# PFLeget/cosmogp

Measured on NVIDIA B200. Metric: gp_fits_per_sec, higher is better.
Workload: dtype f64

## Files before the change

### cosmogp_b200/csrc/cgp_small64.cu

```cuda
#include <atomic>
#include "cgp_internal.h"
#include "cgp_math.cuh"

#include <math.h>
#include <stdlib.h>
#include <type_traits>

#ifndef CGP64_GRID_U
#define CGP64_GRID_U 2
#endif

namespace cgp {
namespace {

constexpr int TILE = 64;
constexpr unsigned FULL = 0xffffffffu;
constexpr double LOG_2PI = 1.8378770664093454835606594728112;
constexpr double LN2 = 0.693147180559945309417232;

__constant__ unsigned char kTri[36] = {
    0x00, 0x10, 0x11, 0x20, 0x21, 0x22, 0x30, 0x31, 0x32, 0x33, 0x40, 0x41, 0x42, 0x43, 0x44,
    0x50, 0x51, 0x52, 0x53, 0x54, 0x55, 0x60, 0x61, 0x62, 0x63, 0x64, 0x65, 0x66,
    0x70, 0x71, 0x72, 0x73, 0x74, 0x75, 0x76, 0x77};

__device__ __forceinline__ void dmma(double& c0, double& c1, double a, double b) {
  asm("mma.sync.aligned.m8n8k4.row.col.f64.f64.f64.f64 {%0,%1}, {%2}, {%3}, {%0,%1};"
      : "+d"(c0), "+d"(c1) : "d"(a), "d"(b));
}
__host__ __device__ constexpr int slot(int i, int j) { return ((i * (i + 1)) >> 1) + j; }
__device__ __forceinline__ int tile_off(int r, int c) {
  const int rho = r ^ ((r >> 1) & 1), sig = (r >> 1) & 2;
  return ((rho * 4 + ((c >> 1) ^ sig)) << 1) + (c & 1);
}

struct Lane {
  int g, t, nat, tr0, tr1;
  __device__ explicit Lane(int lane) {
    g = lane >> 2; t = lane & 3;
    nat = tile_off(g, 2 * t);
    tr0 = tile_off(2 * t, g); tr1 = tile_off(2 * t + 1, g);
  }
};
__device__ __forceinline__ double2 ld_frag(const double* tiles, int s, const Lane& L) {
  return *reinterpret_cast<const double2*>(tiles + s * TILE + L.nat);
}
__device__ __forceinline__ void st_frag(double* tiles, int s, const Lane& L, double v0, double v1) {
  *reinterpret_cast<double2*>(tiles + s * TILE + L.nat) = make_double2(v0, v1);
}
__device__ __forceinline__ double2 ld_frag_t(const double* tiles, int s, const Lane& L) {
  const double* p = tiles + s * TILE;
  return make_double2(p[L.tr0], p[L.tr1]);
}
__device__ __forceinline__ double2 ld_vec2(const double* v, int i) { return *reinterpret_cast<const double2*>(v + i); }
__device__ __forceinline__ double red_t(double v) {
  v += __shfl_xor_sync(FULL, v, 1); v += __shfl_xor_sync(FULL, v, 2); return v;
}
__device__ __forceinline__ double red_g(double v) {
  v += __shfl_xor_sync(FULL, v, 4); v += __shfl_xor_sync(FULL, v, 8); v += __shfl_xor_sync(FULL, v, 16); return v;
}

template <int DIM>
__device__ __forceinline__ double rbf_arg(const Cov& c, double ax, double ay, double bx, double by) {
  const double dx = ax - bx;
  if (DIM == 1) return dx * dx * c.h00;
  const double dy = ay - by;
  return fma(dy * c.h11, dy, fma(dx, c.h00, dy * c.h01) * dx);
}

struct DiagOut { double t0, t1, piv; int badk; };
template <int K>
__device__ __forceinline__ void diag_step(double& a0, double& a1, double& t0, double& t1, double& pivprod, int& badk,
                                          const int g, const int t) {
  constexpr int kc = K >> 1;
  const double ak = (K & 1) ? a1 : a0;
  const double d = __shfl_sync(FULL, ak, K * 4 + kc);
  if (!(d > 0.0) && badk == 0) badk = K + 1;
  const double rinv = cgp_rsqrt(d);
  pivprod *= d;
  const double lg = __shfl_sync(FULL, ak, g * 4 + kc) * rinv;
  const double lc0 = __shfl_sync(FULL, ak, (2 * t) * 4 + kc) * rinv;
  const double lc1 = __shfl_sync(FULL, ak, (2 * t + 1) * 4 + kc) * rinv;
  a0 = fma(-lg, lc0, a0); a1 = fma(-lg, lc1, a1);
  const double tk0 = __shfl_sync(FULL, t0, K * 4 + t) * rinv;
  const double tk1 = __shfl_sync(FULL, t1, K * 4 + t) * rinv;
  const double f = (g > K) ? lg : 0.0;
  const double n0 = fma(-f, tk0, t0), n1 = fma(-f, tk1, t1);
  t0 = (g == K) ? tk0 : n0; t1 = (g == K) ? tk1 : n1;
}
__device__ __noinline__ DiagOut diag_factor_impl(double a0, double a1, int g, int t) {
  double t0 = (g == 2 * t) ? 1.0 : 0.0;
  double t1 = (g == 2 * t + 1) ? 1.0 : 0.0;
  double pivprod = 1.0; int badk = 0;
  diag_step<0>(a0, a1, t0, t1, pivprod, badk, g, t); diag_step<1>(a0, a1, t0, t1, pivprod, badk, g, t);
  diag_step<2>(a0, a1, t0, t1, pivprod, badk, g, t); diag_step<3>(a0, a1, t0, t1, pivprod, badk, g, t);
  diag_step<4>(a0, a1, t0, t1, pivprod, badk, g, t); diag_step<5>(a0, a1, t0, t1, pivprod, badk, g, t);
  diag_step<6>(a0, a1, t0, t1, pivprod, badk, g, t); diag_step<7>(a0, a1, t0, t1, pivprod, badk, g, t);
  DiagOut o; o.t0 = t0; o.t1 = t1; o.piv = pivprod; o.badk = badk;
  return o;
}
__device__ __forceinline__ void diag_factor(double a0, double a1, const Lane& L,
                                            double& t0, double& t1, double& pivprod, int& badk) {
  const DiagOut o = diag_factor_impl(a0, a1, L.g, L.t);
  t0 = o.t0; t1 = o.t1; pivprod = o.piv; badk = o.badk;
}

static unsigned long long* next_ticket(cudaStream_t stream) {
  constexpr unsigned RING = 4096;
  constexpr int MAX_DEV = 16;
  static unsigned long long* ring[MAX_DEV] = {nullptr};
  static std::atomic<unsigned> idx[MAX_DEV];
  int dev = 0;
  if (cudaGetDevice(&dev) != cudaSuccess || dev < 0 || dev >= MAX_DEV) return nullptr;
  if (!ring[dev] && cudaMalloc((void**)&ring[dev], RING * sizeof(unsigned long long)) != cudaSuccess) return nullptr;
  unsigned long long* t = ring[dev] + (idx[dev].fetch_add(1) % RING);
  if (cudaMemsetAsync(t, 0, sizeof(unsigned long long), stream) != cudaSuccess) return nullptr;
  return t;
}

__host__ __device__ constexpr int n_vec64(int task) { return task == TASK_LOO ? 6 : 1; }
__host__ __device__ constexpr bool ktab64(int task, int nb) {
  return task == TASK_LOO || ((task == TASK_PREDICT || task == TASK_PREDICT_U || task == TASK_LL) && nb < 8);
}
#ifndef CGP64_GRID_WPC
#define CGP64_GRID_WPC 1
#endif
__host__ __device__ constexpr int warps_per_cta(int task) { return (task == TASK_PREDICT_F || task == TASK_PREDICT_FU) ? CGP64_GRID_WPC : 1; }

template <int DIM, int TASK, int NB>
__global__ void __launch_bounds__(32 * warps_per_cta(TASK), warps_per_cta(TASK) > 1 ? 16 / warps_per_cta(TASK) :
                                  (TASK == TASK_PREDICT || TASK == TASK_PREDICT_F || TASK == TASK_PREDICT_FU || TASK == TASK_PREDICT_U) ? 12 : 16)
gp64_kernel(const SmallArgs a, unsigned long long* __restrict__ ticket) {
  extern __shared__ __align__(16) double smem[];
  constexpr int WPC = warps_per_cta(TASK);
  const int lane = threadIdx.x & 31, warp = threadIdx.x >> 5;
  const Lane L(lane);
  Cov cov = a.cov;
  constexpr int LD = 8 * NB;
  constexpr int NT = NB * (NB + 1) / 2;
  double* tiles = smem;
  double* px = tiles + NT * TILE + warp * (DIM + 1) * LD;
  double* noise = px + DIM * LD;
  double* vr = tiles + NT * TILE + WPC * (DIM + 1) * LD;
  constexpr bool PF = TASK == TASK_PREDICT_F || TASK == TASK_PREDICT_FU;
  constexpr bool UNI = TASK == TASK_PREDICT_FU || TASK == TASK_PREDICT_U;
  constexpr bool FUSED = TASK == TASK_PREDICT || TASK == TASK_PREDICT_U;
  constexpr bool PRED_LIKE = FUSED || TASK == TASK_FACTOR || PF;
  constexpr bool NEGL = PRED_LIKE;
  double* vz = PRED_LIKE ? vr : vr + LD;
  double* va = PRED_LIKE ? vr : vz + LD;
  double* vd = va + LD;
  double* v1 = vd + LD;
  double* vu = v1 + LD;

  constexpr bool TAB = PF && !UNI && NB == 8 && WPC == 1;
  if (TAB) { exp_table_to_shared(noise, lane); __syncwarp(); }
  constexpr bool KTAB = ktab64(TASK, NB);
  double* const ktab = tiles + NT * TILE + (WPC * (DIM + 1) + n_vec64(TASK)) * LD;
  if (KTAB) { exp_table_to_shared(ktab, lane); __syncwarp(); }
  const int split = (FUSED || PF) ? a.split : 1;
  const int64_t* const part_off = (FUSED || PF) ? a.part_off : nullptr;
  const int64_t n_work = part_off ? a.n_parts : (a.n_obj_dev ? (int64_t)*a.n_obj_dev : a.n_obj) * split;
  __shared__ __align__(8) unsigned long long s_mbar;
  __shared__ long long s_tk[2];
  unsigned mbar_parity = 0;
  if (PF) {
    if (threadIdx.x == 0) {
      asm volatile("mbarrier.init.shared::cta.b64 [%0], 1;" :: "r"((unsigned)__cvta_generic_to_shared(&s_mbar)));
      asm volatile("fence.mbarrier_init.release.cluster;" ::: "memory");
    }
    if (WPC > 1) __syncthreads(); else __syncwarp();
  }

  constexpr int NR = (LD + 31) / 32;
  struct Next { int64_t o0; int n; double x[NR], y2[NR], r[NR], ye[NR]; };
  auto fetch = [&](int64_t w, Next& nx) {
    nx.n = -1;
    if (w >= n_work) return;
    int part, parts;
    const int64_t oi = work_item(part_off, a.n_obj, split, w, part, parts);
    const int64_t b = a.order ? a.order[oi] : oi;
    nx.o0 = a.off[b];
    nx.n = (int)(a.off[b + 1] - nx.o0);
#pragma unroll
    for (int k = 0; k < NR; ++k) {
      const int i = k * 32 + lane;
      const bool in = i < nx.n;
      if (DIM == 1) { nx.x[k] = in ? a.x[nx.o0 + i] : 0.0; nx.y2[k] = 0.0; }
      else { nx.x[k] = in ? a.x[2 * (nx.o0 + i)] : 0.0; nx.y2[k] = in ? a.x[2 * (nx.o0 + i) + 1] : 0.0; }
      if (PF) { nx.ye[k] = 0.0; nx.r[k] = 0.0; continue; }
      nx.ye[k] = (in && a.yerr) ? a.yerr[nx.o0 + i] : 0.0;
      nx.r[k] = in ? (a.y[nx.o0 + i] - (a.y0 ? a.y0[nx.o0 + i] : 0.0)) : 0.0;
    }
  };
  double uni_g0 = 0.0, uni_delta = 0.0, uni_c0 = 1.0, uni_c1 = 1.0, uni_c2 = 1.0, uni_2hd = 0.0;
  if (UNI) {
    uni_g0 = a.xnew[0];
    uni_delta = (a.xnew[a.m_shared - 1] - uni_g0) / (double)(a.m_shared - 1);
    const double k0 = (double)L.g * uni_delta, k1 = (double)(L.g + 8) * uni_delta;
    uni_c0 = cgp_exp(cov.h00 * k0 * k0); uni_c1 = cgp_exp(cov.h00 * k1 * k1);
    const double k2 = (double)(L.g + 16) * uni_delta;
    uni_c2 = cgp_exp(cov.h00 * k2 * k2);
    uni_2hd = 2.0 * cov.h00 * uni_delta;
  }
  int64_t w = blockIdx.x, w_nxt = (int64_t)blockIdx.x + gridDim.x, t_next = 0;
  int it = 0;
  auto advance = [&]() -> int64_t {
    if (WPC > 1) { __syncthreads(); return s_tk[(it++) & 1]; }
    return __shfl_sync(FULL, t_next, 0);
  };
  Next nx;
  fetch(w, nx);
  for (;; w = w_nxt, w_nxt = advance()) {
    if (w >= n_work) break;
    if (threadIdx.x == 0) {
      t_next = (int64_t)atomicAdd(ticket, 1ULL) + 2 * (int64_t)gridDim.x;
      if (WPC > 1) s_tk[it & 1] = t_next;
    }
    int part, parts;
    const int64_t oi = work_item(part_off, a.n_obj, split, w, part, parts);
    const int64_t b = a.order ? a.order[oi] : oi;
    const int64_t o0 = nx.o0;
    const int n = nx.n;
    const int64_t io = a.compact_io ? oi : b;
    if (a.hyp_obj) cov = cov_from_hyp(DIM, a.hyp_obj + io * a.n_hyp, a.nugget_obj ? a.nugget_obj[io] : a.nugget_shared,
                                      a.floor_shared, a.flags);

    __syncwarp();
    double rsum = 0.0;
#pragma unroll
    for (int k = 0; k < NR; ++k) {
      const int i = k * 32 + lane;
      if (i < LD) {
        px[i] = nx.x[k];
        if (DIM == 2) px[LD + i] = nx.y2[k];
        if (!PF) {
          noise[i] = nx.ye[k] * nx.ye[k] + cov.noise_const;
          vr[i] = nx.r[k]; rsum += nx.r[k];
        }
      }
    }
    double xo[NR];
#pragma unroll
    for (int k = 0; k < NR; ++k) xo[k] = UNI ? nx.x[k] : 0.0;
    fetch(w_nxt, nx);
    __syncwarp();
    if (TASK == TASK_LOO) rsum = red_g(red_t(rsum));
    double lp_m = 1.0; int lp_e = 0; int bad = 0;
    const bool want_u = (TASK == TASK_LOO) && (a.loo_mode == 1);
    if (PF) {
      const unsigned mb = (unsigned)__cvta_generic_to_shared(&s_mbar);
      if (threadIdx.x == 0) {
        const unsigned bytes = NT * TILE * 8;
        const double* src = a.fws + b * a.fws_stride;
        asm volatile("fence.proxy.async.shared::cta;" ::: "memory");
        asm volatile("mbarrier.arrive.expect_tx.shared::cta.b64 _, [%0], %1;" :: "r"(mb), "r"(bytes + LD * 8) : "memory");
        asm volatile("cp.async.bulk.shared::cluster.global.mbarrier::complete_tx::bytes [%0], [%1], %2, [%3];"
                     :: "r"((unsigned)__cvta_generic_to_shared(tiles)), "l"(src), "r"(bytes), "r"(mb) : "memory");
        asm volatile("cp.async.bulk.shared::cluster.global.mbarrier::complete_tx::bytes [%0], [%1], %2, [%3];"
                     :: "r"((unsigned)__cvta_generic_to_shared(va)), "l"(src + NT * TILE), "r"((unsigned)(LD * 8)), "r"(mb) : "memory");
      }
      bad = a.info[b];
      unsigned done = 0;
      while (!done) {
        asm volatile("{\n\t.reg .pred p;\n\tmbarrier.try_wait.parity.shared::cta.b64 p, [%1], %2;\n\tselp.u32 %0, 1, 0, p;\n\t}"
                     : "=r"(done) : "r"(mb), "r"(mbar_parity) : "memory");
      }
      mbar_parity ^= 1;
    }
    if (!PF) {

    constexpr int TPP = 4;
#pragma unroll 1
    for (int q = 0; q < NT; q += TPP) {
      double kv[TPP][2];
#pragma unroll
      for (int u = 0; u < TPP; ++u) {
        const int qq = (q + u < NT) ? q + u : q;
        const int ij = kTri[qq];
        const int I = ij >> 4, J = ij & 15;
        const int gi = 8 * I + L.g, cj = 8 * J + 2 * L.t;
        const double xi = px[gi], yi = DIM == 2 ? px[LD + gi] : 0.0;
        const double q0 = rbf_arg<DIM>(cov, xi, yi, px[cj], DIM == 2 ? px[LD + cj] : 0.0);
        const double q1 = rbf_arg<DIM>(cov, xi, yi, px[cj + 1], DIM == 2 ? px[LD + cj + 1] : 0.0);
        double e0 = KTAB ? cgp_exp_tab(q0, ktab) : cgp_exp(q0);
        double e1 = KTAB ? cgp_exp_tab(q1, ktab) : cgp_exp(q1);
        e0 = (gi < n && cj < gi) ? e0 : 0.0;
        e1 = (gi < n && cj + 1 < gi) ? e1 : 0.0;
        const double dg = (gi < n) ? cov.amp_auto + noise[gi] : 1.0;
        kv[u][0] = (cj == gi) ? dg : cov.amp_auto * e0;
        kv[u][1] = (cj + 1 == gi) ? dg : cov.amp_auto * e1;
      }
#pragma unroll
      for (int u = 0; u < TPP; ++u) {
        if (q + u < NT) st_frag(tiles, q + u, L, kv[u][0], kv[u][1]);
      }
    }
    __syncwarp();

#pragma unroll
    for (int J = 0; J < NB; ++J) {
      double s0[NB], s1[NB], u0[NB], u1[NB];
#pragma unroll
      for (int i = 0; i < NB; ++i) { s0[i] = 0.0; s1[i] = 0.0; u0[i] = 0.0; u1[i] = 0.0; }
#pragma unroll
      for (int P = 0; P < J; ++P) {
        const double2 fb = ld_frag(tiles, slot(J, P), L);
        dmma(s0[0], s1[0], fb.x, fb.x); dmma(u0[0], u1[0], fb.y, fb.y);
#pragma unroll
        for (int i = 1; i < NB - J; ++i) {
          const double2 fa = ld_frag(tiles, slot(J + i, P), L);
          dmma(s0[i], s1[i], fa.x, fb.x); dmma(u0[i], u1[i], fa.y, fb.y);
        }
      }
#pragma unroll
      for (int i = 0; i < NB - J; ++i) {
        const double2 kk = ld_frag(tiles, slot(J + i, J), L);
        s0[i] = kk.x - (s0[i] + u0[i]);
        s1[i] = kk.y - (s1[i] + u1[i]);
      }
      double t0, t1;
      {
        double piv; int badk;
        diag_factor(s0[0], s1[0], L, t0, t1, piv, badk);
        st_frag(tiles, slot(J, J), L, t0, t1);
        if (TASK == TASK_LL || TASK == TASK_FACTOR || FUSED) {
          lp_m *= piv;
          const int hi = __double2hiint(lp_m);
          const int e = ((hi >> 20) & 0x7ff) - 1023;
          lp_e += e;
          lp_m = __hiloint2double(hi - (e << 20), __double2loint(lp_m));
        }
        if (badk && bad == 0) bad = 8 * J + badk;
      }
#pragma unroll
      for (int i = 1; i < NB - J; ++i) {
        const double c0 = s0[i], c1 = s1[i];
        s0[i] = 0.0; s1[i] = 0.0; u0[i] = 0.0; u1[i] = 0.0;
        dmma(s0[i], s1[i], c0, t0); dmma(u0[i], u1[i], c1, t1);
      }
#pragma unroll
      for (int i = 1; i < NB - J; ++i) {
        if (NEGL) st_frag(tiles, slot(J + i, J), L, -s0[i] - u0[i], -s1[i] - u1[i]);
        else st_frag(tiles, slot(J + i, J), L, s0[i] + u0[i], s1[i] + u1[i]);
      }
      if (NEGL) {
        double pz = 0.0, pz2 = 0.0;
#pragma unroll
        for (int P = 0; P < J; ++P) {
          const double2 f = ld_frag(tiles, slot(J, P), L);
          const double2 rv = ld_vec2(vr, 8 * P + 2 * L.t);
          pz = fma(f.x, rv.x, pz); pz2 = fma(f.y, rv.y, pz2);
        }
        const double wv = vr[8 * J + L.g] + red_t(pz + pz2);
        double q = t0 * __shfl_sync(FULL, wv, L.t * 8) + t1 * __shfl_sync(FULL, wv, L.t * 8 + 4);
        q = red_t(q);
        if (L.t == 0) vr[8 * J + L.g] = q;
      }
      __syncwarp();
    }

    if (TASK == TASK_LL) {
      double quad = 0.0;
#pragma unroll
      for (int J = 0; J < NB; ++J) {
        double p = 0.0, p2 = 0.0;
#pragma unroll
        for (int P = 0; P < J; ++P) {
          const double2 f = ld_frag(tiles, slot(J, P), L);
          const double2 rv = ld_vec2(vr, 8 * P + 2 * L.t);
          p = fma(f.x, rv.x, p); p2 = fma(f.y, rv.y, p2);
        }
        const double wv = vr[8 * J + L.g] - red_t(p + p2);
        const double2 f = ld_frag(tiles, slot(J, J), L);
        double q = f.x * __shfl_sync(FULL, wv, L.t * 8) + f.y * __shfl_sync(FULL, wv, L.t * 8 + 4);
        q = red_t(q);
        if (L.t == 0) { vr[8 * J + L.g] = q; quad = fma(q, q, quad); }
        __syncwarp();
      }
      quad = red_g(red_t(quad));
      if (lane == 0) {
        a.info[io] = bad;
        const double logdet = log(lp_m) + (double)lp_e * LN2;
        a.ll[io] = bad ? nan("") : -0.5 * (quad + logdet + n * LOG_2PI);
      }
      continue;
    }

    if constexpr (TASK == TASK_LOO) {
#pragma unroll
    for (int I = 1; I < NB; ++I) {
      double s0[NB], s1[NB];
#pragma unroll
      for (int j = 0; j < NB; ++j) { s0[j] = 0.0; s1[j] = 0.0; }
#pragma unroll
      for (int P = 0; P < I; ++P) {
        const double2 fb = ld_frag(tiles, slot(I, P), L);
#pragma unroll
        for (int J = 0; J <= P; ++J) {
          const double2 fa = (J == P) ? ld_frag_t(tiles, slot(P, P), L) : ld_frag(tiles, slot(P, J), L);
          dmma(s0[J], s1[J], fa.x, fb.x); dmma(s0[J], s1[J], fa.y, fb.y);
        }
      }
      const double2 ft = ld_frag(tiles, slot(I, I), L);
#pragma unroll
      for (int J = 0; J < I; ++J) {
        double r0 = 0.0, r1 = 0.0, e0 = 0.0, e1 = 0.0;
        dmma(r0, r1, s0[J], ft.x); dmma(e0, e1, s1[J], ft.y);
        s0[J] = -(r0 + e0); s1[J] = -(r1 + e1);
      }
#pragma unroll
      for (int J = 0; J < I; ++J) st_frag(tiles, slot(I, J), L, s0[J], s1[J]);
      __syncwarp();
    }
#pragma unroll
    for (int I = 1; I < NB; ++I) {
      double2 v[NB];
#pragma unroll
      for (int J = 0; J < I; ++J) v[J] = ld_frag_t(tiles, slot(I, J), L);
      __syncwarp();
#pragma unroll
      for (int J = 0; J < I; ++J) st_frag(tiles, slot(I, J), L, v[J].x, v[J].y);
    }
    __syncwarp();

#pragma unroll
    for (int I = 0; I < NB; ++I) {
      double p = 0.0, p2 = 0.0, p1 = 0.0;
#pragma unroll
      for (int J = 0; J <= I; ++J) {
        const double2 f = ld_frag(tiles, slot(I, J), L);
        const double2 rv = ld_vec2(vr, 8 * J + 2 * L.t);
        p = fma(f.x, rv.x, p); p2 = fma(f.y, rv.y, p2);
        if (TASK == TASK_LOO) { p1 += f.x; p1 += f.y; }
      }
      p = red_t(p + p2);
      if (L.t == 0) vz[8 * I + L.g] = p;
      if (TASK == TASK_LOO) { p1 = red_t(p1); if (L.t == 0) v1[8 * I + L.g] = (8 * I + L.g < n) ? p1 : 0.0; }
    }
    __syncwarp();
#pragma unroll
    for (int J = 0; J < NB; ++J) {
      double pa0 = 0.0, pa1 = 0.0, pd0 = 0.0, pd1 = 0.0, pu0 = 0.0, pu1 = 0.0;
#pragma unroll
      for (int I = J; I < NB; ++I) {
        const double2 f = ld_frag(tiles, slot(I, J), L);
        const double zi = vz[8 * I + L.g];
        pa0 = fma(f.x, zi, pa0); pa1 = fma(f.y, zi, pa1);
        if (TASK == TASK_LOO) {
          const bool in = 8 * I + L.g < n;
          pd0 = in ? fma(f.x, f.x, pd0) : pd0; pd1 = in ? fma(f.y, f.y, pd1) : pd1;
          const double ui = v1[8 * I + L.g];
          pu0 = fma(f.x, ui, pu0); pu1 = fma(f.y, ui, pu1);
        }
      }
      pa0 = red_g(pa0); pa1 = red_g(pa1);
      if (L.g == 0) { va[8 * J + 2 * L.t] = pa0; va[8 * J + 2 * L.t + 1] = pa1; }
      if (TASK == TASK_LOO) {
        pd0 = red_g(pd0); pd1 = red_g(pd1); pu0 = red_g(pu0); pu1 = red_g(pu1);
        if (L.g == 0) {
          vd[8 * J + 2 * L.t] = pd0; vd[8 * J + 2 * L.t + 1] = pd1;
          vu[8 * J + 2 * L.t] = pu0; vu[8 * J + 2 * L.t + 1] = pu1;
        }
      }
    }
    __syncwarp();
    }
    if (lane == 0 && part == 0) a.info[b] = bad;
    }

    if (FUSED && a.ll && part == 0) {
      double quad = 0.0;
#pragma unroll
      for (int i0 = 0; i0 < LD; i0 += 32) { const int i = i0 + lane; if (i < LD) quad = fma(vz[i], vz[i], quad); }
      quad = red_g(red_t(quad));
      if (lane == 0) {
        const double logdet = log(lp_m) + (double)lp_e * LN2;
        a.ll[b] = bad ? nan("") : -0.5 * (quad + logdet + n * LOG_2PI);
      }
      __syncwarp();
    }
    if (TASK == TASK_FACTOR) {
      if (a.ll) {
        double quad = 0.0;
#pragma unroll
        for (int i0 = 0; i0 < LD; i0 += 32) { const int i = i0 + lane; if (i < LD) quad = fma(vz[i], vz[i], quad); }
        quad = red_g(red_t(quad));
        if (lane == 0) {
          const double logdet = log(lp_m) + (double)lp_e * LN2;
          a.ll[b] = bad ? nan("") : -0.5 * (quad + logdet + n * LOG_2PI);
        }
      }
      double* dst = a.fws + b * a.fws_stride;
#pragma unroll 4
      for (int q = 0; q < NT; ++q)
        reinterpret_cast<double2*>(dst + q * TILE)[lane] = reinterpret_cast<const double2*>(tiles + q * TILE)[lane];
#pragma unroll
      for (int i0 = 0; i0 < LD; i0 += 32) { const int i = i0 + lane; if (i < LD) dst[NT * TILE + i] = va[i]; }
      continue;
    }

    if (TASK == TASK_LOO) {
      const double rho = cov.amp_cross / cov.amp_auto;
      const double amp_star = cov.amp_auto + cov.nugget2;
#pragma unroll
      for (int i0 = 0; i0 < LD; i0 += 32) {
        const int i = i0 + lane;
        if (i < n) {
          const double d = vd[i], r = vr[i];
          const double yv = a.y[o0 + i];
          const double m = a.y0 ? a.y0[o0 + i] : 0.0;
          const double ye = a.yerr ? a.yerr[o0 + i] : 0.0;
          double pr = m + rho * (r - va[i] / d);
          if (want_u) {
            const double delta = (rsum - r) / (double)(n - 1);
            pr += delta - delta * rho * (1.0 - vu[i] / d);
          }
          double pv = fabs(amp_star - rho * rho * (cov.amp_auto + noise[i] - 1.0 / d));
          double res = pr - yv;
          double pl = res / sqrt(ye * ye + pv + cov.nugget2);
          if (bad) { pr = nan(""); pv = pr; res = pr; pl = pr; }
          if (a.pred) a.pred[o0 + i] = pr;
          if (a.pvar) a.pvar[o0 + i] = pv;
          if (a.resid) a.resid[o0 + i] = res;
          if (a.pull) a.pull[o0 + i] = pl;
        }
      }
      continue;
    }

    if (FUSED || PF) {
      constexpr int UB = CGP64_GRID_U;
      constexpr bool TAIL3 = UNI && PF && UB == 2 && WPC == 1;
      constexpr int UMAX = TAIL3 ? 3 : UB;
      const int64_t g0 = a.goff ? a.goff[b] : 0;
      const int64_t m_pts = a.goff ? (a.goff[b + 1] - g0) : a.m_shared;
      const int64_t out0 = a.goff ? g0 : b * a.m_shared;
      const int64_t n_rb = (m_pts + 7) >> 3;
      const double amp_star = cov.amp_auto + cov.nugget2;
      double pgx[UMAX], pgy[UMAX], pny0[UMAX];
      auto grid_fetch = [&](int64_t rb) {
#pragma unroll
        for (int u = 0; u < UMAX; ++u) {
          const int64_t m = 8 * (rb + u) + L.g;
          const bool lv = m < m_pts;
          pgx[u] = 0.0; pgy[u] = 0.0;
          if (lv && !UNI) {
            if (DIM == 1) pgx[u] = a.xnew[g0 + m];
            else { pgx[u] = a.xnew[2 * (g0 + m)]; pgy[u] = a.xnew[2 * (g0 + m) + 1]; }
          }
          pny0[u] = (lv && a.new_y0) ? (a.new_y0_diff ? a.new_y0[m] + a.new_y0_diff[b] : a.new_y0[out0 + m]) : 0.0;
        }
      };
      const int64_t rb0 = (int64_t)(part * WPC + warp) * UB, rbs = (int64_t)parts * WPC * UB;
      grid_fetch(rb0);
      auto pass = [&](auto Uc, const int64_t rb, const int64_t rb_next) {
        constexpr int U = decltype(Uc)::value;
        int64_t mi[U]; bool live[U]; double gx[U], gy[U], ny0[U];
#pragma unroll
        for (int u = 0; u < U; ++u) {
          mi[u] = 8 * (rb + u) + L.g;
          live[u] = mi[u] < m_pts;
          gx[u] = pgx[u]; gy[u] = pgy[u]; ny0[u] = pny0[u];
        }
        grid_fetch(rb_next);
        double acc0[U][NB], acc1[U][NB];
        if constexpr (UNI) {
          double2* anch = reinterpret_cast<double2*>(px);
          const bool second = (U == 1) && (rbs == 1) && (rb & 1);
          (void)second;
          if (!second) {
          __syncwarp();
          const double gj0 = fma((double)(8 * rb), uni_delta, uni_g0);
#pragma unroll
          for (int k = 0; k < NR; ++k) {
            const int c = k * 32 + lane;
            const double uu = gj0 - xo[k];
            double ea = cgp_exp(cov.h00 * uu * uu), rr = cgp_exp(uni_2hd * uu);
            ea = (c < n && ea > 0.0) ? ea : 0.0;
            rr = (ea > 0.0) ? rr : 0.0;
            if (c < LD) anch[c] = make_double2(ea, rr);
          }
          __syncwarp();
          }
          const bool b1 = L.g & 1, b2 = L.g & 2, b4 = L.g & 4;
#pragma unroll
          for (int P = 0; P < NB; ++P) {
            const int c0 = 8 * P + 2 * L.t, c1 = c0 + 1;
            const double2 A0 = anch[c0], A1 = anch[c1];
            const double r02 = A0.y * A0.y, r04 = r02 * r02, r08 = r04 * r04;
            const double r12 = A1.y * A1.y, r14 = r12 * r12, r18 = r14 * r14;
            double p0 = b1 ? A0.y : 1.0, p1 = b1 ? A1.y : 1.0;
            if (b2) { p0 *= r02; p1 *= r12; }
            if (b4) { p0 *= r04; p1 *= r14; }
            const double t0 = A0.x * p0, t1 = A1.x * p1;
            if constexpr (U >= 2) {
              const double s0 = t0 * r08, s1 = t1 * r18;
              acc0[0][P] = t0 * uni_c0; acc0[1][P] = s0 * uni_c1; acc1[0][P] = t1 * uni_c0; acc1[1][P] = s1 * uni_c1;
              if constexpr (U == 3) { acc0[2][P] = (s0 * r08) * uni_c2; acc1[2][P] = (s1 * r18) * uni_c2; }
            } else {
              const double cs = second ? uni_c1 : uni_c0;
              acc0[0][P] = (second ? t0 * r08 : t0) * cs; acc1[0][P] = (second ? t1 * r18 : t1) * cs;
            }
          }
        } else {
#pragma unroll
        for (int P = 0; P < NB; ++P) {
          const int c0 = 8 * P + 2 * L.t, c1 = c0 + 1;
          const double2 xx = ld_vec2(px, c0);
          const double x0 = xx.x, x1 = xx.y;
          double y0c = 0.0, y1c = 0.0;
          if (DIM == 2) { const double2 yy = ld_vec2(px + LD, c0); y0c = yy.x; y1c = yy.y; }
#pragma unroll
          for (int u = 0; u < U; ++u) {
            double e0 = TAB ? cgp_exp_tab(rbf_arg<DIM>(cov, gx[u], gy[u], x0, y0c), noise) : cgp_exp(rbf_arg<DIM>(cov, gx[u], gy[u], x0, y0c));
            double e1 = TAB ? cgp_exp_tab(rbf_arg<DIM>(cov, gx[u], gy[u], x1, y1c), noise) : cgp_exp(rbf_arg<DIM>(cov, gx[u], gy[u], x1, y1c));
            e0 = (live[u] && c0 < n) ? e0 : 0.0;
            e1 = (live[u] && c1 < n) ? e1 : 0.0;
            acc0[u][P] = e0; acc1[u][P] = e1;
          }
        }
        }
        double pm[U], pm2[U], vs[U], vs2[U];
#pragma unroll
        for (int u = 0; u < U; ++u) { pm[u] = 0.0; pm2[u] = 0.0; vs[u] = 0.0; vs2[u] = 0.0; }
#pragma unroll
        for (int P = 0; P < NB; ++P) {
          const double2 ft = ld_frag(tiles, slot(P, P), L);
          const double2 zz = ld_vec2(va, 8 * P + 2 * L.t);
#pragma unroll
          for (int u = 0; u < U; ++u) {
            double v0 = 0.0, v1 = 0.0;
            dmma(v0, v1, acc0[u][P], ft.x); dmma(v0, v1, acc1[u][P], ft.y);
            acc0[u][P] = v0; acc1[u][P] = v1;
            if (TASK == TASK_PREDICT && a.vout && live[u])
              *reinterpret_cast<double2*>(a.vout + (out0 + mi[u]) * LD + 8 * P + 2 * L.t) = make_double2(v0, v1);
            pm[u] = fma(v0, zz.x, pm[u]); pm2[u] = fma(v1, zz.y, pm2[u]);
            vs[u] = fma(v0, v0, vs[u]); vs2[u] = fma(v1, v1, vs2[u]);
          }
#pragma unroll
          for (int J = P + 1; J < NB; ++J) {
            const double2 fb = ld_frag(tiles, slot(J, P), L);
#pragma unroll
            for (int u = 0; u < U; ++u) dmma(acc0[u][J], acc1[u][J], acc0[u][P], fb.x);
#pragma unroll
            for (int u = 0; u < U; ++u) dmma(acc0[u][J], acc1[u][J], acc1[u][P], fb.y);
          }
        }
#pragma unroll
        for (int u = 0; u < U; ++u) {
          double vv = vs[u], vv2 = vs2[u];
          const double pmt = red_t(pm[u] + pm2[u]);
          vv = red_t(vv + vv2);
          if (live[u] && L.t == 0) {
            double mean = fma(cov.amp_cross, pmt, ny0[u]);
            double var = fma(-cov.amp_cross * cov.amp_cross, vv, amp_star);
            if (bad) { mean = nan(""); var = mean; }
            a.mean[out0 + mi[u]] = mean;
            if (a.var) a.var[out0 + mi[u]] = var;
          }
        }
      };
      if (TAIL3 && rbs == UB) {
        for (int64_t rb = rb0; rb < n_rb;) {
          const int64_t left = n_rb - rb;
          if (left == 1 || left == 2 || left == 4) { pass(std::integral_constant<int, UB>{}, rb, rb + UB); rb += UB; }
          else { pass(std::integral_constant<int, UMAX>{}, rb, rb + UMAX); rb += UMAX; }
        }
      } else {
        for (int64_t rb = rb0; rb < n_rb; rb += rbs) pass(std::integral_constant<int, UB>{}, rb, rb + rbs);
      }
    }
  }
}


template <int B, int E, class F>
__device__ __forceinline__ void static_for(F&& f) {
  if constexpr (B < E) { f(std::integral_constant<int, B>{}); static_for<B + 1, E>(f); }
}

constexpr int kPhys[8][8][8] = {
    {{0, 0, 0, 0, 0, 0, 0, 0}, {0, 0, 0, 0, 0, 0, 0, 0}, {0, 0, 0, 0, 0, 0, 0, 0}, {0, 0, 0, 0, 0, 0, 0, 0}, {0, 0, 0, 0, 0, 0, 0, 0}, {0, 0, 0, 0, 0, 0, 0, 0}, {0, 0, 0, 0, 0, 0, 0, 0}, {0, 0, 0, 0, 0, 0, 0, 0}},
    {{0, 0, 0, 0, 0, 0, 0, 0}, {1, 0, 0, 0, 0, 0, 0, 0}, {0, 0, 0, 0, 0, 0, 0, 0}, {0, 0, 0, 0, 0, 0, 0, 0}, {0, 0, 0, 0, 0, 0, 0, 0}, {0, 0, 0, 0, 0, 0, 0, 0}, {0, 0, 0, 0, 0, 0, 0, 0}, {0, 0, 0, 0, 0, 0, 0, 0}},
    {{0, 0, 0, 0, 0, 0, 0, 0}, {1, 0, 0, 0, 0, 0, 0, 0}, {2, 3, 0, 0, 0, 0, 0, 0}, {0, 0, 0, 0, 0, 0, 0, 0}, {0, 0, 0, 0, 0, 0, 0, 0}, {0, 0, 0, 0, 0, 0, 0, 0}, {0, 0, 0, 0, 0, 0, 0, 0}, {0, 0, 0, 0, 0, 0, 0, 0}},
    {{0, 0, 0, 0, 0, 0, 0, 0}, {1, 0, 0, 0, 0, 0, 0, 0}, {2, 4, 0, 0, 0, 0, 0, 0}, {3, 5, 1, 0, 0, 0, 0, 0}, {0, 0, 0, 0, 0, 0, 0, 0}, {0, 0, 0, 0, 0, 0, 0, 0}, {0, 0, 0, 0, 0, 0, 0, 0}, {0, 0, 0, 0, 0, 0, 0, 0}},
    {{0, 0, 0, 0, 0, 0, 0, 0}, {1, 0, 0, 0, 0, 0, 0, 0}, {2, 5, 0, 0, 0, 0, 0, 0}, {3, 6, 1, 0, 0, 0, 0, 0}, {4, 7, 8, 2, 0, 0, 0, 0}, {0, 0, 0, 0, 0, 0, 0, 0}, {0, 0, 0, 0, 0, 0, 0, 0}, {0, 0, 0, 0, 0, 0, 0, 0}},
    {{0, 0, 0, 0, 0, 0, 0, 0}, {1, 0, 0, 0, 0, 0, 0, 0}, {2, 6, 0, 0, 0, 0, 0, 0}, {3, 7, 1, 0, 0, 0, 0, 0}, {4, 8, 10, 2, 0, 0, 0, 0}, {5, 9, 11, 6, 1, 0, 0, 0}, {0, 0, 0, 0, 0, 0, 0, 0}, {0, 0, 0, 0, 0, 0, 0, 0}},
    {{0, 0, 0, 0, 0, 0, 0, 0}, {1, 0, 0, 0, 0, 0, 0, 0}, {2, 7, 0, 0, 0, 0, 0, 0}, {3, 8, 1, 0, 0, 0, 0, 0}, {4, 9, 12, 2, 0, 0, 0, 0}, {5, 10, 13, 7, 1, 0, 0, 0}, {6, 11, 14, 15, 3, 2, 0, 0}, {0, 0, 0, 0, 0, 0, 0, 0}},
    {{0, 0, 0, 0, 0, 0, 0, 0}, {1, 0, 0, 0, 0, 0, 0, 0}, {2, 8, 0, 0, 0, 0, 0, 0}, {3, 9, 1, 0, 0, 0, 0, 0}, {4, 10, 14, 2, 0, 0, 0, 0}, {5, 11, 15, 8, 1, 0, 0, 0}, {6, 12, 16, 18, 3, 2, 0, 0}, {7, 13, 17, 19, 9, 4, 1, 0}}};
constexpr int kPhysSlots[8] = {1, 2, 4, 6, 9, 12, 16, 20};

template <int DIM, int NB>
__global__ void __launch_bounds__(32, 16)
gp64_ll_kernel(const SmallArgs a, unsigned long long* __restrict__ ticket) {
  extern __shared__ __align__(16) double smem[];
  const int lane = threadIdx.x;
  const Lane L(lane);
  Cov cov = a.cov;
  constexpr int LD = 8 * NB;
  constexpr int NSLOT = kPhysSlots[NB - 1];
  double* tiles = smem;
  double* px = tiles + NSLOT * TILE;
  double* noise = px + DIM * LD;
  double* vr = noise + LD;
  double* etab = vr + LD;
  exp_table_to_shared(etab, lane);
  __syncwarp();
  const int64_t n_work = a.n_obj_dev ? (int64_t)*a.n_obj_dev : a.n_obj;

  constexpr int NR = (LD + 31) / 32;
  struct Next { int64_t b, io; int n; double x[NR], y2[NR], r[NR], ye[NR]; };
  auto fetch = [&](int64_t w, Next& nx) {
    nx.n = -1; nx.b = 0; nx.io = 0;
    if (w >= n_work) return;
    nx.b = a.order ? a.order[w] : w;
    nx.io = a.compact_io ? w : nx.b;
    const int64_t o0 = a.off[nx.b];
    nx.n = (int)(a.off[nx.b + 1] - o0);
#pragma unroll
    for (int k = 0; k < NR; ++k) {
      const int i = k * 32 + lane;
      const bool in = i < nx.n;
      if (DIM == 1) { nx.x[k] = in ? a.x[o0 + i] : 0.0; nx.y2[k] = 0.0; }
      else { nx.x[k] = in ? a.x[2 * (o0 + i)] : 0.0; nx.y2[k] = in ? a.x[2 * (o0 + i) + 1] : 0.0; }
      nx.ye[k] = (in && a.yerr) ? a.yerr[o0 + i] : 0.0;
      nx.r[k] = in ? (a.y[o0 + i] - (a.y0 ? a.y0[o0 + i] : 0.0)) : 0.0;
    }
  };
  int64_t w = blockIdx.x, w_nxt = (int64_t)blockIdx.x + gridDim.x, t_next = 0;
  Next nx;
  fetch(w, nx);
  for (;; w = w_nxt, w_nxt = __shfl_sync(FULL, t_next, 0)) {
    if (w >= n_work) break;
    if (lane == 0) t_next = (int64_t)atomicAdd(ticket, 1ULL) + 2 * (int64_t)gridDim.x;
    const int64_t io = nx.io, nx_b = nx.b;
    const int n = nx.n;
    if (a.hyp_obj) cov = cov_from_hyp(DIM, a.hyp_obj + io * a.n_hyp, a.nugget_obj ? a.nugget_obj[io] : a.nugget_shared,
                                      a.floor_shared, a.flags);
    __syncwarp();
#pragma unroll
    for (int k = 0; k < NR; ++k) {
      const int i = k * 32 + lane;
      if (i < LD) {
        px[i] = nx.x[k];
        if (DIM == 2) px[LD + i] = nx.y2[k];
        noise[i] = nx.ye[k] * nx.ye[k] + cov.noise_const;
        vr[i] = nx.r[k];
      }
    }
    fetch(w_nxt, nx);
    __syncwarp();

    double lp_m = 1.0, quad = 0.0; int lp_e = 0; int bad = 0;
    constexpr int NTF = NB * (NB + 1) / 2;
    double* const fdst = a.fws ? a.fws + nx_b * a.fws_stride : nullptr;
    static_for<0, NB>([&](auto Jc) {
      constexpr int J = decltype(Jc)::value;
      constexpr int NTJ = NB - J;
      double k0[NTJ], k1[NTJ];
      static_for<0, NTJ>([&](auto ic) {
        constexpr int i = decltype(ic)::value;
        const int gi = 8 * (J + i) + L.g, cj = 8 * J + 2 * L.t;
        const double xi = px[gi], yi = DIM == 2 ? px[LD + gi] : 0.0;
        double e0 = cgp_exp_tab(rbf_arg<DIM>(cov, xi, yi, px[cj], DIM == 2 ? px[LD + cj] : 0.0), etab);
        double e1 = cgp_exp_tab(rbf_arg<DIM>(cov, xi, yi, px[cj + 1], DIM == 2 ? px[LD + cj + 1] : 0.0), etab);
        e0 = (gi < n && cj < gi) ? e0 : 0.0;
        e1 = (gi < n && cj + 1 < gi) ? e1 : 0.0;
        const double dg = (gi < n) ? cov.amp_auto + noise[gi] : 1.0;
        k0[i] = (i == 0 && cj == gi) ? dg : cov.amp_auto * e0;
        k1[i] = (i == 0 && cj + 1 == gi) ? dg : cov.amp_auto * e1;
      });
      double s0[NTJ], s1[NTJ], u0[NTJ], u1[NTJ];
      static_for<0, NTJ>([&](auto ic) { constexpr int i = decltype(ic)::value; s0[i] = 0.0; s1[i] = 0.0; u0[i] = 0.0; u1[i] = 0.0; });
      static_for<0, J>([&](auto Pc) {
        constexpr int P = decltype(Pc)::value;
        const double2 fb = ld_frag(tiles, kPhys[NB - 1][J][P], L);
        dmma(s0[0], s1[0], fb.x, fb.x); dmma(u0[0], u1[0], fb.y, fb.y);
        static_for<1, NTJ>([&](auto ic) {
          constexpr int i = decltype(ic)::value;
          const double2 fa = ld_frag(tiles, kPhys[NB - 1][J + i][P], L);
          dmma(s0[i], s1[i], fa.x, fb.x); dmma(u0[i], u1[i], fa.y, fb.y);
        });
      });
      static_for<0, NTJ>([&](auto ic) {
        constexpr int i = decltype(ic)::value;
        s0[i] = k0[i] - (s0[i] + u0[i]); s1[i] = k1[i] - (s1[i] + u1[i]);
      });
      double t0, t1;
      {
        double piv; int badk;
        diag_factor(s0[0], s1[0], L, t0, t1, piv, badk);
        lp_m *= piv;
        const int hi = __double2hiint(lp_m);
        const int e = ((hi >> 20) & 0x7ff) - 1023;
        lp_e += e;
        lp_m = __hiloint2double(hi - (e << 20), __double2loint(lp_m));
        if (badk && bad == 0) bad = 8 * J + badk;
      }
      if constexpr (NTJ > 1) {
        static_for<1, NTJ>([&](auto ic) {
          constexpr int i = decltype(ic)::value;
          const double c0 = s0[i], c1 = s1[i];
          s0[i] = 0.0; s1[i] = 0.0; u0[i] = 0.0; u1[i] = 0.0;
          dmma(s0[i], s1[i], c0, t0); dmma(u0[i], u1[i], c1, t1);
        });
        static_for<1, NTJ>([&](auto ic) {
          constexpr int i = decltype(ic)::value;
          constexpr int ps = kPhys[NB - 1][J + i][J];
          st_frag(tiles, ps, L, s0[i] + u0[i], s1[i] + u1[i]);
        });
      }
      double pz = 0.0, pz2 = 0.0;
      static_for<0, J>([&](auto Pc) {
        constexpr int P = decltype(Pc)::value;
        const double2 f = ld_frag(tiles, kPhys[NB - 1][J][P], L);
        const double2 rv = ld_vec2(vr, 8 * P + 2 * L.t);
        pz = fma(f.x, rv.x, pz); pz2 = fma(f.y, rv.y, pz2);
        if (fdst) *reinterpret_cast<double2*>(fdst + slot(J, P) * TILE + L.nat) = make_double2(-f.x, -f.y);
      });
      if (fdst) *reinterpret_cast<double2*>(fdst + slot(J, J) * TILE + L.nat) = make_double2(t0, t1);
      const double wv = vr[8 * J + L.g] - red_t(pz + pz2);
      double q = t0 * __shfl_sync(FULL, wv, L.t * 8) + t1 * __shfl_sync(FULL, wv, L.t * 8 + 4);
      q = red_t(q);
      if (L.t == 0) { vr[8 * J + L.g] = q; quad = fma(q, q, quad); }
      __syncwarp();
    });
    quad = red_g(red_t(quad));
    if (fdst) {
#pragma unroll
      for (int i0 = 0; i0 < LD; i0 += 32) { const int i = i0 + lane; if (i < LD) fdst[NTF * TILE + i] = vr[i]; }
    }
    if (lane == 0) {
      a.info[io] = bad;
      const double logdet = log(lp_m) + (double)lp_e * LN2;
      if (a.ll) a.ll[io] = bad ? nan("") : -0.5 * (quad + logdet + n * LOG_2PI);
    }
  }
}


template <int DIM, int NB>
int launch64_ll(const SmallArgs& a, cudaStream_t stream) {
  auto kern = gp64_ll_kernel<DIM, NB>;
  const size_t smem = ((size_t)kPhysSlots[NB - 1] * TILE + (size_t)(DIM + 2) * 8 * NB + 64) * sizeof(double);
  static int sm_counts[16] = {0}, per_sms[16] = {0};
  int dev = 0;
  if (cudaGetDevice(&dev) != cudaSuccess || dev < 0 || dev >= 16) return (int)cudaErrorInvalidDevice;
  int& sm_count = sm_counts[dev]; int& per_sm = per_sms[dev];
  if (!sm_count) cudaDeviceGetAttribute(&sm_count, cudaDevAttrMultiProcessorCount, dev);
  if (!per_sm) {
    cudaError_t e = cudaFuncSetAttribute(kern, cudaFuncAttributeMaxDynamicSharedMemorySize, (int)smem);
    if (e != cudaSuccess) return (int)e;
    int occ = 0;
    e = cudaOccupancyMaxActiveBlocksPerMultiprocessor(&occ, kern, 32, smem);
    if (e != cudaSuccess) return (int)e;
    if (occ < 1) return (int)cudaErrorInvalidConfiguration;
    per_sm = occ > 16 ? 16 : occ;
  }
  static int cap = -1;
  if (cap < 0) { const char* e = getenv("CGP_GP64_PER_SM"); cap = e ? atoi(e) : 0; }
  int64_t grid = (int64_t)sm_count * ((cap > 0 && cap < per_sm) ? cap : per_sm);
  if (grid > a.n_obj) grid = a.n_obj;
  if (grid < 1) return 0;
  unsigned long long* ticket = next_ticket(stream);
  if (!ticket) return (int)cudaErrorMemoryAllocation;
  kern<<<(unsigned)grid, 32, smem, stream>>>(a, ticket);
  count_launch();
  return (int)cudaGetLastError();
}

template <int DIM, int TASK, int NB>
int launch64(const SmallArgs& a, cudaStream_t stream) {
  static int compact = -1;
  if (compact < 0) { const char* e = getenv("CGP_LL_COMPACT"); compact = (e && !atoi(e)) ? 0 : 1; }
  static int fcompact = -1;
  if (fcompact < 0) { const char* e = getenv("CGP_FACTOR_COMPACT"); fcompact = (e && !atoi(e)) ? 0 : 1; }
  if ((TASK == TASK_LL && compact) || (TASK == TASK_FACTOR && fcompact)) return launch64_ll<DIM, NB>(a, stream);
  auto kern = gp64_kernel<DIM, TASK, NB>;
  constexpr int WPC = warps_per_cta(TASK);
  const size_t smem = ((size_t)(NB * (NB + 1) / 2) * TILE + (size_t)(WPC * (DIM + 1) + n_vec64(TASK)) * 8 * NB
                       + (ktab64(TASK, NB) ? 64 : 0)) * sizeof(double);
  static int sm_counts[16] = {0}, per_sms[16] = {0};
  int dev = 0;
  if (cudaGetDevice(&dev) != cudaSuccess || dev < 0 || dev >= 16) return (int)cudaErrorInvalidDevice;
  int& sm_count = sm_counts[dev]; int& per_sm = per_sms[dev];
  if (!sm_count) cudaDeviceGetAttribute(&sm_count, cudaDevAttrMultiProcessorCount, dev);
  if (!per_sm) {
    cudaError_t e = cudaFuncSetAttribute(kern, cudaFuncAttributeMaxDynamicSharedMemorySize, (int)smem);
    if (e != cudaSuccess) return (int)e;
    int occ = 0;
    e = cudaOccupancyMaxActiveBlocksPerMultiprocessor(&occ, kern, 32 * WPC, smem);
    if (e != cudaSuccess) return (int)e;
    if (occ < 1) return (int)cudaErrorInvalidConfiguration;
    per_sm = occ;
  }
  constexpr bool GRID_TASK = TASK == TASK_PREDICT || TASK == TASK_PREDICT_F || TASK == TASK_PREDICT_FU || TASK == TASK_PREDICT_U;
  const int64_t n_work = !GRID_TASK ? a.n_obj : a.part_off ? a.n_parts : a.n_obj * a.split;
  static int cap = -1;
  if (cap < 0) { const char* e = getenv("CGP_GP64_PER_SM"); cap = e ? atoi(e) : 0; }
  int64_t grid = (int64_t)sm_count * ((cap > 0 && cap < per_sm) ? cap : per_sm);
  if (grid > n_work) grid = n_work;
  if (grid < 1) return 0;
  unsigned long long* ticket = next_ticket(stream);
  if (!ticket) return (int)cudaErrorMemoryAllocation;
  kern<<<(unsigned)grid, 32 * WPC, smem, stream>>>(a, ticket);
  count_launch();
  return (int)cudaGetLastError();
}

template <int DIM, int TASK>
int launch64_nb(int nb, const SmallArgs& a, cudaStream_t stream) {
  switch (nb) {
    case 1: return launch64<DIM, TASK, 1>(a, stream);
    case 2: return launch64<DIM, TASK, 2>(a, stream);
    case 3: return launch64<DIM, TASK, 3>(a, stream);
    case 4: return launch64<DIM, TASK, 4>(a, stream);
    case 5: return launch64<DIM, TASK, 5>(a, stream);
    case 6: return launch64<DIM, TASK, 6>(a, stream);
    case 7: return launch64<DIM, TASK, 7>(a, stream);
    case 8: return launch64<DIM, TASK, 8>(a, stream);
  }
  return (int)cudaErrorInvalidValue;
}

}

#ifndef CGP64_DIM
#error "compile with -DCGP64_DIM=1|2 -DCGP64_TASK=0|1|2|4|5|6|7"
#endif
#define CGP64_CAT2(a, b, c, d) a##b##c##d
#define CGP64_CAT(a, b, c, d) CGP64_CAT2(a, b, c, d)
int CGP64_CAT(launch_small64_d, CGP64_DIM, _t, CGP64_TASK)(int nb, const SmallArgs& a, cudaStream_t stream) {
  return launch64_nb<CGP64_DIM, CGP64_TASK>(nb, a, stream);
}

}
```

Before: 31.49 million.

## Precompute uniform-grid cross-kernel power rows in shared memory and defer scaling

For uniform-grid prediction tasks, the per-column exponential powers (ea*rr^g for g=0..7, plus rr^8) are now computed once when the anchor is built and stored as nine swizzled rows in shared memory. Each MMA lane then loads its value directly instead of rebuilding products with per-lane branches. The per-row constant factors move out of the accumulator initialisation into the final mean/variance scaling, read from a small shared table, and exponentials use a table-based exp. The failure flag and per-object y0 offset are prefetched with the next work item, so the loop no longer does those dependent global loads. The cost is more shared memory per warp, which may lower occupancy, plus extra shared stores during anchor construction.

```diff
diff --git a/cosmogp_b200/csrc/cgp_small64.cu b/cosmogp_b200/csrc/cgp_small64.cu
--- a/cosmogp_b200/csrc/cgp_small64.cu
+++ b/cosmogp_b200/csrc/cgp_small64.cu
@@ -121,6 +121,10 @@
 __host__ __device__ constexpr bool ktab64(int task, int nb) {
   return task == TASK_LOO || ((task == TASK_PREDICT || task == TASK_PREDICT_U || task == TASK_LL) && nb < 8);
 }
+__host__ __device__ constexpr bool uni64(int task) { return task == TASK_PREDICT_FU || task == TASK_PREDICT_U; }
+constexpr int UNI_ROWS = 9;
+__host__ __device__ constexpr int px_rows64(int task, int dim) { return uni64(task) ? UNI_ROWS : dim + 1; }
+__host__ __device__ constexpr bool etab64(int task, int nb) { return ktab64(task, nb) || uni64(task); }
 #ifndef CGP64_GRID_WPC
 #define CGP64_GRID_WPC 1
 #endif
@@ -138,11 +142,12 @@
   constexpr int LD = 8 * NB;
   constexpr int NT = NB * (NB + 1) / 2;
   double* tiles = smem;
-  double* px = tiles + NT * TILE + warp * (DIM + 1) * LD;
+  constexpr int PXR = px_rows64(TASK, DIM);
+  double* px = tiles + NT * TILE + warp * PXR * LD;
   double* noise = px + DIM * LD;
-  double* vr = tiles + NT * TILE + WPC * (DIM + 1) * LD;
+  double* vr = tiles + NT * TILE + WPC * PXR * LD;
   constexpr bool PF = TASK == TASK_PREDICT_F || TASK == TASK_PREDICT_FU;
-  constexpr bool UNI = TASK == TASK_PREDICT_FU || TASK == TASK_PREDICT_U;
+  constexpr bool UNI = uni64(TASK);
   constexpr bool FUSED = TASK == TASK_PREDICT || TASK == TASK_PREDICT_U;
   constexpr bool PRED_LIKE = FUSED || TASK == TASK_FACTOR || PF;
   constexpr bool NEGL = PRED_LIKE;
@@ -155,8 +160,8 @@
   constexpr bool TAB = PF && !UNI && NB == 8 && WPC == 1;
   if (TAB) { exp_table_to_shared(noise, lane); __syncwarp(); }
   constexpr bool KTAB = ktab64(TASK, NB);
-  double* const ktab = tiles + NT * TILE + (WPC * (DIM + 1) + n_vec64(TASK)) * LD;
-  if (KTAB) { exp_table_to_shared(ktab, lane); __syncwarp(); }
+  double* const ktab = tiles + NT * TILE + (WPC * PXR + n_vec64(TASK)) * LD;
+  if (etab64(TASK, NB)) { exp_table_to_shared(ktab, lane); __syncwarp(); }
   const int split = (FUSED || PF) ? a.split : 1;
   const int64_t* const part_off = (FUSED || PF) ? a.part_off : nullptr;
   const int64_t n_work = part_off ? a.n_parts : (a.n_obj_dev ? (int64_t)*a.n_obj_dev : a.n_obj) * split;
@@ -172,7 +177,7 @@
   }
 
   constexpr int NR = (LD + 31) / 32;
-  struct Next { int64_t o0; int n; double x[NR], y2[NR], r[NR], ye[NR]; };
+  struct Next { int64_t o0; int n, bad; double ydiff, x[NR], y2[NR], r[NR], ye[NR]; };
   auto fetch = [&](int64_t w, Next& nx) {
     nx.n = -1;
     if (w >= n_work) return;
@@ -181,6 +186,8 @@
     const int64_t b = a.order ? a.order[oi] : oi;
     nx.o0 = a.off[b];
     nx.n = (int)(a.off[b + 1] - nx.o0);
+    nx.bad = PF ? a.info[b] : 0;
+    nx.ydiff = ((FUSED || PF) && a.new_y0 && a.new_y0_diff) ? a.new_y0_diff[b] : 0.0;
 #pragma unroll
     for (int k = 0; k < NR; ++k) {
       const int i = k * 32 + lane;
@@ -192,15 +199,15 @@
       nx.r[k] = in ? (a.y[nx.o0 + i] - (a.y0 ? a.y0[nx.o0 + i] : 0.0)) : 0.0;
     }
   };
-  double uni_g0 = 0.0, uni_delta = 0.0, uni_c0 = 1.0, uni_c1 = 1.0, uni_c2 = 1.0, uni_2hd = 0.0;
+  double uni_g0 = 0.0, uni_delta = 0.0, uni_2hd = 0.0;
+  double* const uni_c = ktab + 64;
   if (UNI) {
     uni_g0 = a.xnew[0];
     uni_delta = (a.xnew[a.m_shared - 1] - uni_g0) / (double)(a.m_shared - 1);
-    const double k0 = (double)L.g * uni_delta, k1 = (double)(L.g + 8) * uni_delta;
-    uni_c0 = cgp_exp(cov.h00 * k0 * k0); uni_c1 = cgp_exp(cov.h00 * k1 * k1);
-    const double k2 = (double)(L.g + 16) * uni_delta;
-    uni_c2 = cgp_exp(cov.h00 * k2 * k2);
+    const double kd = (double)lane * uni_delta;
+    if (lane < 24) uni_c[lane] = cgp_exp(cov.h00 * kd * kd);
     uni_2hd = 2.0 * cov.h00 * uni_delta;
+    __syncwarp();
   }
   int64_t w = blockIdx.x, w_nxt = (int64_t)blockIdx.x + gridDim.x, t_next = 0;
   int it = 0;
@@ -242,10 +249,12 @@
     double xo[NR];
 #pragma unroll
     for (int k = 0; k < NR; ++k) xo[k] = UNI ? nx.x[k] : 0.0;
+    const double ydiff = nx.ydiff;
+    int bad = nx.bad;
     fetch(w_nxt, nx);
     __syncwarp();
     if (TASK == TASK_LOO) rsum = red_g(red_t(rsum));
-    double lp_m = 1.0; int lp_e = 0; int bad = 0;
+    double lp_m = 1.0; int lp_e = 0;
     const bool want_u = (TASK == TASK_LOO) && (a.loo_mode == 1);
     if (PF) {
       const unsigned mb = (unsigned)__cvta_generic_to_shared(&s_mbar);
@@ -259,7 +268,6 @@
         asm volatile("cp.async.bulk.shared::cluster.global.mbarrier::complete_tx::bytes [%0], [%1], %2, [%3];"
                      :: "r"((unsigned)__cvta_generic_to_shared(va)), "l"(src + NT * TILE), "r"((unsigned)(LD * 8)), "r"(mb) : "memory");
       }
-      bad = a.info[b];
       unsigned done = 0;
       while (!done) {
         asm volatile("{\n\t.reg .pred p;\n\tmbarrier.try_wait.parity.shared::cta.b64 p, [%1], %2;\n\tselp.u32 %0, 1, 0, p;\n\t}"
@@ -548,7 +556,7 @@
             if (DIM == 1) pgx[u] = a.xnew[g0 + m];
             else { pgx[u] = a.xnew[2 * (g0 + m)]; pgy[u] = a.xnew[2 * (g0 + m) + 1]; }
           }
-          pny0[u] = (lv && a.new_y0) ? (a.new_y0_diff ? a.new_y0[m] + a.new_y0_diff[b] : a.new_y0[out0 + m]) : 0.0;
+          pny0[u] = (lv && a.new_y0) ? a.new_y0[a.new_y0_diff ? m : out0 + m] : 0.0;
         }
       };
       const int64_t rb0 = (int64_t)(part * WPC + warp) * UB, rbs = (int64_t)parts * WPC * UB;
@@ -564,10 +572,10 @@
         }
         grid_fetch(rb_next);
         double acc0[U][NB], acc1[U][NB];
+        const bool second = UNI && (U == 1) && (rbs == 1) && (rb & 1);
         if constexpr (UNI) {
-          double2* anch = reinterpret_cast<double2*>(px);
-          const bool second = (U == 1) && (rbs == 1) && (rb & 1);
-          (void)second;
+          double* pw = px;
+          constexpr int SWZ = (NB & 1) ? 0 : 8;
           if (!second) {
           __syncwarp();
           const double gj0 = fma((double)(8 * rb), uni_delta, uni_g0);
@@ -575,31 +583,32 @@
           for (int k = 0; k < NR; ++k) {
             const int c = k * 32 + lane;
             const double uu = gj0 - xo[k];
-            double ea = cgp_exp(cov.h00 * uu * uu), rr = cgp_exp(uni_2hd * uu);
+            double ea = cgp_exp_tab(cov.h00 * uu * uu, ktab), rr = cgp_exp_tab(uni_2hd * uu, ktab);
             ea = (c < n && ea > 0.0) ? ea : 0.0;
             rr = (ea > 0.0) ? rr : 0.0;
-            if (c < LD) anch[c] = make_double2(ea, rr);
+            if (c < LD) {
+              const double r2 = rr * rr, r4 = r2 * r2;
+              const double e1 = ea * rr, e2 = ea * r2, e3 = e1 * r2;
+              const double e[8] = {ea, e1, e2, e3, ea * r4, e1 * r4, e2 * r4, e3 * r4};
+#pragma unroll
+              for (int g = 0; g < 8; ++g) pw[g * LD + (c ^ ((g & 1) * SWZ))] = e[g];
+              pw[(UNI_ROWS - 1) * LD + c] = r4 * r4;
+            }
           }
           __syncwarp();
           }
-          const bool b1 = L.g & 1, b2 = L.g & 2, b4 = L.g & 4;
 #pragma unroll
           for (int P = 0; P < NB; ++P) {
-            const int c0 = 8 * P + 2 * L.t, c1 = c0 + 1;
-            const double2 A0 = anch[c0], A1 = anch[c1];
-            const double r02 = A0.y * A0.y, r04 = r02 * r02, r08 = r04 * r04;
-            const double r12 = A1.y * A1.y, r14 = r12 * r12, r18 = r14 * r14;
-            double p0 = b1 ? A0.y : 1.0, p1 = b1 ? A1.y : 1.0;
-            if (b2) { p0 *= r02; p1 *= r12; }
-            if (b4) { p0 *= r04; p1 *= r14; }
-            const double t0 = A0.x * p0, t1 = A1.x * p1;
+            const int c0 = 8 * P + 2 * L.t;
+            const double2 r8 = ld_vec2(pw + (UNI_ROWS - 1) * LD, c0);
+            const double2 er = ld_vec2(pw + L.g * LD, c0 ^ ((L.g & 1) * SWZ));
+            const double t0 = er.x, t1 = er.y;
             if constexpr (U >= 2) {
-              const double s0 = t0 * r08, s1 = t1 * r18;
-              acc0[0][P] = t0 * uni_c0; acc0[1][P] = s0 * uni_c1; acc1[0][P] = t1 * uni_c0; acc1[1][P] = s1 * uni_c1;
-              if constexpr (U == 3) { acc0[2][P] = (s0 * r08) * uni_c2; acc1[2][P] = (s1 * r18) * uni_c2; }
+              const double s0 = t0 * r8.x, s1 = t1 * r8.y;
+              acc0[0][P] = t0; acc0[1][P] = s0; acc1[0][P] = t1; acc1[1][P] = s1;
+              if constexpr (U == 3) { acc0[2][P] = s0 * r8.x; acc1[2][P] = s1 * r8.y; }
             } else {
-              const double cs = second ? uni_c1 : uni_c0;
-              acc0[0][P] = (second ? t0 * r08 : t0) * cs; acc1[0][P] = (second ? t1 * r18 : t1) * cs;
+              acc0[0][P] = second ? t0 * r8.x : t0; acc1[0][P] = second ? t1 * r8.y : t1;
             }
           }
         } else {
@@ -652,8 +661,9 @@
           const double pmt = red_t(pm[u] + pm2[u]);
           vv = red_t(vv + vv2);
           if (live[u] && L.t == 0) {
-            double mean = fma(cov.amp_cross, pmt, ny0[u]);
-            double var = fma(-cov.amp_cross * cov.amp_cross, vv, amp_star);
+            const double ac = UNI ? cov.amp_cross * uni_c[L.g + 8 * (second ? 1 : u)] : cov.amp_cross;
+            double mean = fma(ac, pmt, a.new_y0_diff ? ny0[u] + ydiff : ny0[u]);
+            double var = fma(-ac * ac, vv, amp_star);
             if (bad) { mean = nan(""); var = mean; }
             a.mean[out0 + mi[u]] = mean;
             if (a.var) a.var[out0 + mi[u]] = var;
@@ -878,8 +888,8 @@
   if ((TASK == TASK_LL && compact) || (TASK == TASK_FACTOR && fcompact)) return launch64_ll<DIM, NB>(a, stream);
   auto kern = gp64_kernel<DIM, TASK, NB>;
   constexpr int WPC = warps_per_cta(TASK);
-  const size_t smem = ((size_t)(NB * (NB + 1) / 2) * TILE + (size_t)(WPC * (DIM + 1) + n_vec64(TASK)) * 8 * NB
-                       + (ktab64(TASK, NB) ? 64 : 0)) * sizeof(double);
+  const size_t smem = ((size_t)(NB * (NB + 1) / 2) * TILE + (size_t)(WPC * px_rows64(TASK, DIM) + n_vec64(TASK)) * 8 * NB
+                       + (etab64(TASK, NB) ? 64 : 0) + (uni64(TASK) ? 24 : 0)) * sizeof(double);
   static int sm_counts[16] = {0}, per_sms[16] = {0};
   int dev = 0;
   if (cudaGetDevice(&dev) != cudaSuccess || dev < 0 || dev >= 16) return (int)cudaErrorInvalidDevice;
```

New measurement: 33.09 million, median of 6. 5.1% higher.
